# uzh-rpg/dagr

Hardware: AMD Instinct MI355X
Metric: events_per_sec (higher is better)
Workload: dtype f32; 1 GPU; dagr-s + --use_image --img_net resnet50, 640x480 synthetic S-uniform, B=8 windows/step x 100000 events (50 ms each), r=7, K=16, events->graph->GNN(+image fusion)->decoded head outputs->confidence mask + NMS (device); image_branch=in-line, engines=3

## Files before the change

dagr_amd/csrc/gemm_split_bf16.hip:

```cpp
#include <algorithm>
#include <type_traits>

#include "common.hpp"

namespace dagr {
namespace {

constexpr int kKT = 32;
constexpr int kNPad = 128;

typedef __bf16 bf16x8 __attribute__((ext_vector_type(8)));
typedef float f32x4 __attribute__((ext_vector_type(4)));
typedef unsigned u32x2 __attribute__((ext_vector_type(2)));

struct Geo {
    int mode;
    int H, W, C, s, Ho, Wo;
};

struct Args {
    const float *A;
    const unsigned short *Wp;
    const float *bias, *R;
    float *D;
    int64_t M, lda, ldr, ldd;
    int K, N, Npad, act, n_tiles_n, n_blocks;
    Geo g;
};

__device__ __forceinline__ unsigned short bf16_bits(__bf16 v) { return __builtin_bit_cast(unsigned short, v); }

__device__ __forceinline__ void split3(float a, unsigned short &p1, unsigned short &p2, unsigned short &p3) {
    const __bf16 b1 = (__bf16)a;
    const float r1 = a - (float)b1;
    const __bf16 b2 = (__bf16)r1;
    const float r2 = r1 - (float)b2;
    const __bf16 b3 = (__bf16)r2;
    p1 = bf16_bits(b1);
    p2 = bf16_bits(b2);
    p3 = bf16_bits(b3);
}

__device__ __forceinline__ void split3x2(float a0, float a1, unsigned &p1, unsigned &p2, unsigned &p3) {
    typedef float f32x2 __attribute__((ext_vector_type(2)));
    typedef __bf16 bf16x2 __attribute__((ext_vector_type(2)));
    auto widen = [](unsigned u) {
        return f32x2{__builtin_bit_cast(float, u << 16), __builtin_bit_cast(float, u & 0xffff0000u)};
    };
    const f32x2 v = {a0, a1};
    p1 = __builtin_bit_cast(unsigned, __builtin_convertvector(v, bf16x2));
    const f32x2 r1 = v - widen(p1);
    p2 = __builtin_bit_cast(unsigned, __builtin_convertvector(r1, bf16x2));
    const f32x2 r2 = r1 - widen(p2);
    p3 = __builtin_bit_cast(unsigned, __builtin_convertvector(r2, bf16x2));
}

__device__ __forceinline__ int swz(int r, int c) { return r * kKT + ((c ^ (((r >> 3) & 1) * 3)) << 3); }

__global__ __launch_bounds__(256) void k_split_pack(const float *__restrict__ Wt, int K, int N, int Npad,
                                                    unsigned short *__restrict__ out) {
    const int64_t total = (int64_t)K * Npad;
    for (int64_t i = (int64_t)blockIdx.x * blockDim.x + threadIdx.x; i < total; i += (int64_t)gridDim.x * blockDim.x) {
        const int k = (int)(i / Npad), n = (int)(i - (int64_t)k * Npad);
        unsigned short p[3] = {0, 0, 0};
        if (n < N) split3(Wt[(int64_t)k * N + n], p[0], p[1], p[2]);
        const int kt = k / kKT, kk = k - kt * kKT;
#pragma unroll
        for (int q = 0; q < 3; q++) out[((int64_t)kt * 3 + q) * Npad * kKT + swz(n, kk >> 3) + (kk & 7)] = p[q];
    }
}

template <int N>
__device__ __forceinline__ void wait_all_barrier(f32x4 (&ra)[2][N]) {
    if constexpr (N == 1)
        asm volatile("s_waitcnt vmcnt(0) lgkmcnt(0)" : "+v"(ra[0][0]), "+v"(ra[1][0])::"memory");
    else
        asm volatile("s_waitcnt vmcnt(0) lgkmcnt(0)" : "+v"(ra[0][0]), "+v"(ra[0][1]), "+v"(ra[1][0]), "+v"(ra[1][1])::"memory");
    __builtin_amdgcn_s_barrier();
    asm volatile("" ::: "memory");
}

constexpr int waves_per_simd(int BN, int WN) { return WN == 4 ? 4 : BN == 128 ? 2 : 3; }

template <int MI, int BN, int MODE, int WN = 2>
__global__ __launch_bounds__(128 * WN, waves_per_simd(BN, WN)) void k_gemm_split(const Args a) {
    constexpr int BM = 32 * MI;
    constexpr int NT = 128 * WN;
    constexpr int NI = BN / (16 * WN);
    constexpr int AI = BM * 8 / NT;
    constexpr int kStage = 3 * (BM + BN) * kKT;
    constexpr int kPieces = 3 * BN / 16 / (2 * WN);
    static_assert(AI >= 1 && AI * NT == BM * 8 && kPieces * 2 * WN * 16 == 3 * BN && NI >= 1, "tile does not divide among the waves");
    __shared__ __attribute__((aligned(1024))) unsigned short lds[2 * kStage];

    const int orig = blockIdx.x, xcd = orig & 7, q8 = a.n_blocks >> 3, r8 = a.n_blocks & 7;
    const int lid = (xcd < r8 ? xcd * (q8 + 1) : r8 * (q8 + 1) + (xcd - r8) * q8) + (orig >> 3);
    const int nt = lid % a.n_tiles_n, mt = lid / a.n_tiles_n;
    const int64_t m0 = (int64_t)mt * BM;
    const int n0 = nt * BN;

    const int t = threadIdx.x, lane = t & 63, wave = t >> 6;
    const int wm = wave / WN, wn = wave % WN;

    constexpr int kRS = NT / 8;
    const int r0 = t >> 3, c4 = t & 7;
    int64_t rowoff[MODE == 1 ? AI : 1];
    int ryx[MODE == 2 ? AI : 1];
    const int64_t mrow0 = m0 + r0;
    rowoff[0] = (mrow0 < a.M ? mrow0 : 0) * a.lda;
    ryx[0] = 0;
#pragma unroll
    for (int i = 0; i < AI; i++) {
        const int64_t m = mrow0 + kRS * i;
        const int64_t mm = m < a.M ? m : 0;
        if (MODE == 1) {
            const int64_t b = mm / ((int64_t)a.g.Ho * a.g.Wo);
            const int rem = (int)(mm - b * (int64_t)a.g.Ho * a.g.Wo);
            const int yo = rem / a.g.Wo, xo = rem - yo * a.g.Wo;
            rowoff[MODE == 1 ? i : 0] = ((b * a.g.H + (int64_t)yo * a.g.s) * a.g.W + (int64_t)xo * a.g.s) * a.lda;
        } else if (MODE == 2) {
            ryx[MODE == 2 ? i : 0] = (int)((mm / a.g.W) % a.g.H) << 16 | (int)(mm % a.g.W);
        }
    }

    static_assert(AI == 1 || AI == 2, "wait_all_barrier names the register sets");
    f32x4 ra[2][AI];
    unsigned okmask[2] = {0, 0};

    auto gload = [&](auto set, int kt) {
        constexpr int S = decltype(set)::value;
        const int k0 = kt * kKT;
        int c0 = k0, dy = 0, dx = 0;
        int64_t toff = 0;
        if (MODE == 2) {
            const int tap = k0 / a.g.C;
            c0 = k0 - tap * a.g.C;
            dy = tap / 3 - 1;
            dx = tap - (tap / 3) * 3 - 1;
            toff = (int64_t)(dy * a.g.W + dx) * a.lda;
        }
        okmask[S] = 0;
#pragma unroll
        for (int i = 0; i < AI; i++) {
            bool ok = mrow0 + kRS * i < a.M;
            if (MODE == 2) {
                const int yx = ryx[MODE == 2 ? i : 0];
                ok = ok && (unsigned)((yx >> 16) + dy) < (unsigned)a.g.H && (unsigned)((yx & 0xffff) + dx) < (unsigned)a.g.W;
            }
            const int64_t off = MODE == 1 ? rowoff[MODE == 1 ? i : 0] : rowoff[0] + (int64_t)(kRS * i) * a.lda;
            const float *p = ok ? a.A + off + toff + c0 + c4 * 4 : a.A;
            ra[S][i] = *reinterpret_cast<const f32x4 *>(p);
            okmask[S] |= (ok ? 1u : 0u) << i;
        }
    };

    auto lwrite = [&](auto set, int s) {
        constexpr int S = decltype(set)::value;
        unsigned short *const ldsA = lds + s * kStage;
#pragma unroll
        for (int i = 0; i < AI; i++) {
            const bool ok = (okmask[S] >> i) & 1u;
            const f32x4 v = ok ? ra[S][i] : f32x4{0.f, 0.f, 0.f, 0.f};
            unsigned lo[3], hi[3];
            split3x2(v[0], v[1], lo[0], lo[1], lo[2]);
            split3x2(v[2], v[3], hi[0], hi[1], hi[2]);
#pragma unroll
            for (int q = 0; q < 3; q++) {
                const u32x2 u = {lo[q], hi[q]};
                *reinterpret_cast<u32x2 *>(ldsA + q * BM * kKT + swz(r0 + kRS * i, c4 >> 1) + (c4 & 1) * 4) = u;
            }
        }
    };

    const char *const wsrc = reinterpret_cast<const char *>(a.Wp) + ((int64_t)n0 * kKT) * 2 + lane * 16;
    auto wload = [&](int kt, int s) {
#pragma unroll
        for (int j = 0; j < kPieces; j++) {
            const int piece = wave * kPieces + j, p = piece / (BN / 16), sub = piece - p * (BN / 16);
            const char *src = wsrc + (((int64_t)kt * 3 + p) * a.Npad * kKT + sub * 16 * kKT) * 2;
            unsigned short *dst = lds + s * kStage + (3 * BM + p * BN + sub * 16) * kKT;
            __builtin_amdgcn_global_load_lds((const __attribute__((address_space(1))) void *)src,
                                             (__attribute__((address_space(3))) void *)dst, 16, 0, 0);
        }
    };

    f32x4 acc[MI][NI];
#pragma unroll
    for (int mi = 0; mi < MI; mi++)
#pragma unroll
        for (int ni = 0; ni < NI; ni++) acc[mi][ni] = f32x4{0.f, 0.f, 0.f, 0.f};

    const int frag = swz(lane & 15, lane >> 4);
    const int fragA = (wm * 16 * MI) * kKT + frag;
    const int fragW = (3 * BM + wn * (BN / WN)) * kKT + frag;

    const int n_kt = a.K / kKT;
    const std::integral_constant<int, 0> set0;
    const std::integral_constant<int, 1> set1;

    auto multiply = [&](const unsigned short *st) {
        bf16x8 bw[3][NI], av[MI][3];
#pragma unroll
        for (int p = 0; p < 3; p++)
#pragma unroll
            for (int ni = 0; ni < NI; ni++)
                bw[p][ni] = *reinterpret_cast<const bf16x8 *>(st + fragW + (p * BN + ni * 16) * kKT);
#pragma unroll
        for (int mi = 0; mi < MI; mi++)
#pragma unroll
            for (int p = 0; p < 3; p++) av[mi][p] = *reinterpret_cast<const bf16x8 *>(st + fragA + (p * BM + mi * 16) * kKT);
        const f32x4 zero = {0.f, 0.f, 0.f, 0.f};
#pragma unroll
        for (int mi = 0; mi < MI; mi++) {
            f32x4 ts[NI];
#pragma unroll
            for (int ni = 0; ni < NI; ni++) ts[ni] = __builtin_amdgcn_mfma_f32_16x16x32_bf16(bw[2][ni], av[mi][0], zero, 0, 0, 0);
#pragma unroll
            for (int ni = 0; ni < NI; ni++) ts[ni] = __builtin_amdgcn_mfma_f32_16x16x32_bf16(bw[0][ni], av[mi][2], ts[ni], 0, 0, 0);
#pragma unroll
            for (int ni = 0; ni < NI; ni++) ts[ni] = __builtin_amdgcn_mfma_f32_16x16x32_bf16(bw[1][ni], av[mi][1], ts[ni], 0, 0, 0);
#pragma unroll
            for (int ni = 0; ni < NI; ni++) ts[ni] = __builtin_amdgcn_mfma_f32_16x16x32_bf16(bw[1][ni], av[mi][0], ts[ni], 0, 0, 0);
#pragma unroll
            for (int ni = 0; ni < NI; ni++) ts[ni] = __builtin_amdgcn_mfma_f32_16x16x32_bf16(bw[0][ni], av[mi][1], ts[ni], 0, 0, 0);
#pragma unroll
            for (int ni = 0; ni < NI; ni++) ts[ni] = __builtin_amdgcn_mfma_f32_16x16x32_bf16(bw[0][ni], av[mi][0], ts[ni], 0, 0, 0);
#pragma unroll
            for (int ni = 0; ni < NI; ni++) acc[mi][ni] += ts[ni];
        }
    };

    auto slice = [&](auto cur, auto nxt, int kt) {
        constexpr int S = decltype(cur)::value;
        gload(cur, kt + 2 < n_kt ? kt + 2 : n_kt - 1);
        wload(kt + 1, S ^ 1);
        __builtin_amdgcn_sched_barrier(0);
        multiply(lds + S * kStage);
        lwrite(nxt, S ^ 1);
#pragma unroll
        for (int i = 0; i < 6 * MI * NI; i++) {
            __builtin_amdgcn_sched_group_barrier(0x008, 1, 0);
            __builtin_amdgcn_sched_group_barrier(0x002, 3, 0);
        }
        wait_all_barrier(ra);
    };

    gload(set0, 0);
    gload(set1, n_kt > 1 ? 1 : 0);
    wload(0, 0);
    lwrite(set0, 0);
    wait_all_barrier(ra);
    int kt = 0;
    for (; kt + 2 < n_kt; kt += 2) {
        slice(set0, set1, kt);
        slice(set1, set0, kt + 1);
    }
    if (kt + 1 < n_kt) {
        slice(set0, set1, kt);
        kt++;
    }
    multiply(lds + (kt & 1) * kStage);

#pragma unroll
    for (int mi = 0; mi < MI; mi++) {
        const int64_t m = m0 + wm * 16 * MI + mi * 16 + (lane & 15);
        if (m >= a.M) continue;
#pragma unroll
        for (int ni = 0; ni < NI; ni++) {
            const int n = n0 + wn * (BN / WN) + ni * 16 + (lane >> 4) * 4;
            if (n >= a.N) continue;
            f32x4 v = acc[mi][ni];
            if (a.bias) {
                const float4 b = *reinterpret_cast<const float4 *>(a.bias + n);
                v += f32x4{b.x, b.y, b.z, b.w};
            }
            if (a.R) {
                const float4 r = *reinterpret_cast<const float4 *>(a.R + m * a.ldr + n);
                v += f32x4{r.x, r.y, r.z, r.w};
            }
            if (a.act) v = f32x4{fmaxf(v[0], 0.f), fmaxf(v[1], 0.f), fmaxf(v[2], 0.f), fmaxf(v[3], 0.f)};
            *reinterpret_cast<float4 *>(a.D + m * a.ldd + n) = make_float4(v[0], v[1], v[2], v[3]);
        }
    }
}

inline bool aligned16(const void *p) { return ((uintptr_t)p & 15) == 0; }

template <int MI, int BN, int MODE, int WN = 2>
int launch_tile(Args &a, hipStream_t stream) {
    a.n_tiles_n = (int)ceil_div(a.N, BN);
    const int64_t blocks = ceil_div(a.M, 32 * MI) * a.n_tiles_n;
    DAGR_CHECK_ARG(blocks < ((int64_t)1 << 31), "too many tiles");
    a.n_blocks = (int)blocks;
    k_gemm_split<MI, BN, MODE, WN><<<(unsigned)blocks, 128 * WN, 0, stream>>>(a);
    DAGR_CHECK_LAUNCH();
    return DAGR_OK;
}

template <int MODE>
int launch(Args &a, int variant, hipStream_t stream) {
    if (variant == 0) {
        const int64_t cus = device_cu_count();
        if (MODE != 2 && a.K <= 512 && a.N % 128 == 0 && ceil_div(a.M, 64) * (a.N / 128) >= 4 * cus)
            variant = DAGR_SPLIT_64X128_W8;
        else
            variant = ceil_div(a.M, 64) * ceil_div(a.N, 64) >= 2 * cus ? DAGR_SPLIT_64X64 : DAGR_SPLIT_32X64;
    }
    switch (variant) {
        case DAGR_SPLIT_64X128: return launch_tile<2, 128, MODE>(a, stream);
        case DAGR_SPLIT_32X128: return launch_tile<1, 128, MODE>(a, stream);
        case DAGR_SPLIT_64X64: return launch_tile<2, 64, MODE>(a, stream);
        case DAGR_SPLIT_32X64: return launch_tile<1, 64, MODE>(a, stream);
        case DAGR_SPLIT_64X128_W8: return launch_tile<2, 128, MODE, 4>(a, stream);
    }
    set_error("split-bf16 GEMM: unknown variant");
    return DAGR_ERR_INVALID_ARG;
}

inline int unsupported(const char *fn, const char *what) {
    set_error(std::string(fn) + ": " + what);
    return DAGR_ERR_UNSUPPORTED;
}

}
}

using namespace dagr;

extern "C" size_t dagr_gemm_split_bf16_packed_bytes(int32_t K, int32_t N) {
    if (K < kKT || K % kKT != 0 || N < 16 || N % 16 != 0) return 0;
    return (size_t)K * 3 * align_up((size_t)N, kNPad) * sizeof(unsigned short);
}

extern "C" int dagr_gemm_split_bf16_pack(const float *Wt, int32_t K, int32_t N, void *packed, size_t packed_bytes,
                                         void *stream) {
    DAGR_CHECK_ARG(K >= 1 && N >= 1, "bad sizes");
    if (K % kKT != 0) return unsupported(__func__, "K is not a multiple of the K-tile (32)");
    if (N % 16 != 0) return unsupported(__func__, "N is not a multiple of 16");
    DAGR_CHECK_ARG(Wt && packed, "NULL pointer");
    DAGR_CHECK_ARG(aligned16(packed), "packed is not 16-byte aligned");
    DAGR_CHECK_ARG(packed_bytes >= dagr_gemm_split_bf16_packed_bytes(K, N), "packed buffer too small");
    const int Npad = (int)align_up((size_t)N, kNPad);
    const int64_t blocks = std::min<int64_t>(ceil_div((int64_t)K * Npad, 256), 256 * 16);
    k_split_pack<<<(unsigned)blocks, 256, 0, (hipStream_t)stream>>>(Wt, K, N, Npad, (unsigned short *)packed);
    DAGR_CHECK_LAUNCH();
    return DAGR_OK;
}

namespace {
#define SPLIT_CHECK(cond, msg)                                     \
    do {                                                           \
        if (!(cond)) {                                             \
            set_error(std::string(fn) + ": " + (msg));             \
            return DAGR_ERR_INVALID_ARG;                           \
        }                                                          \
    } while (0)

int check_common(const char *fn, const float *A, int64_t M, int32_t K, int64_t lda, const void *packed, int32_t N,
                 const float *bias, const float *R, int64_t ldr, int32_t act, float *D, int64_t ldd, int32_t code,
                 int32_t max_code, bool &done) {
    done = true;
    SPLIT_CHECK(M >= 0 && K >= 1 && N >= 1 && ldd >= N && (!R || ldr >= N) && (act == 0 || act == 1) && code >= 0 &&
                    code <= max_code,
                "bad sizes");
    if (K % kKT != 0) return unsupported(fn, "K (C of a 3x3) is not a multiple of the K-tile (32)");
    if (N % 16 != 0) return unsupported(fn, "N is not a multiple of 16");
    if (M == 0) return DAGR_OK;
    SPLIT_CHECK(A && packed && D, "NULL pointer");
    SPLIT_CHECK((const float *)D != A, "D aliases A");
    SPLIT_CHECK((const float *)D != R, "D aliases R");
    SPLIT_CHECK(lda % 4 == 0 && ldd % 4 == 0 && (!R || ldr % 4 == 0), "row strides must be multiples of 4 floats");
    SPLIT_CHECK(aligned16(A) && aligned16(packed) && aligned16(D) && aligned16(bias) && aligned16(R),
                "pointers must be 16-byte aligned");
    done = false;
    return DAGR_OK;
}

int gemm_entry(const char *fn, const float *A, int64_t M, int32_t K, int64_t lda, const void *packed, int32_t N,
               const float *bias, const float *R, int64_t ldr, int32_t act, float *D, int64_t ldd, int32_t B, int32_t H,
               int32_t W, int32_t stride, int32_t code, int32_t max_code, void *stream) {
    bool done;
    const int rc = check_common(fn, A, M, K, lda, packed, N, bias, R, ldr, act, D, ldd, code, max_code, done);
    if (done) return rc;
    SPLIT_CHECK(lda >= K && stride >= 1, "bad sizes");
    Args a{A, (const unsigned short *)packed, bias, R, D, M, lda, R ? ldr : 0, ldd, K, N, (int)align_up((size_t)N, kNPad), act,
           0, 0, Geo{0, 0, 0, K, 1, 0, 0}};
    if (stride == 1) return launch<0>(a, code, (hipStream_t)stream);
    SPLIT_CHECK(B >= 1 && H >= 1 && W >= 1, "bad image sizes");
    const int Ho = (H - 1) / stride + 1, Wo = (W - 1) / stride + 1;
    SPLIT_CHECK(M == (int64_t)B * Ho * Wo, "M is not B * ceil(H / stride) * ceil(W / stride)");
    a.g = Geo{1, H, W, K, stride, Ho, Wo};
    return launch<1>(a, code, (hipStream_t)stream);
}

int conv3x3_entry(const char *fn, const float *X, int32_t B, int32_t H, int32_t W, int32_t C, int64_t ldx, const void *packed,
                  int32_t N, const float *bias, const float *R, int64_t ldr, int32_t act, float *D, int64_t ldd, int32_t code,
                  int32_t max_code, void *stream) {
    SPLIT_CHECK(B >= 0 && H >= 1 && W >= 1 && C >= 1 && ldx >= C, "bad sizes");
    const int64_t M = (int64_t)B * H * W;
    bool done;
    const int rc = check_common(fn, X, M, C, ldx, packed, N, bias, R, ldr, act, D, ldd, code, max_code, done);
    if (done) return rc;
    SPLIT_CHECK((int64_t)C * 9 < ((int64_t)1 << 31), "C too large");
    Args a{X, (const unsigned short *)packed, bias, R, D, M, ldx, R ? ldr : 0, ldd, 9 * C, N, (int)align_up((size_t)N, kNPad), act,
           0, 0, Geo{2, H, W, C, 1, H, W}};
    return launch<2>(a, code, (hipStream_t)stream);
}
#undef SPLIT_CHECK
}

extern "C" int dagr_gemm_split_bf16(const float *A, int64_t M, int32_t K, int64_t lda, const void *packed, int32_t N,
                                    const float *bias, const float *R, int64_t ldr, int32_t act, float *D, int64_t ldd,
                                    int32_t B, int32_t H, int32_t W, int32_t stride, int32_t tile, void *stream) {
    return gemm_entry(__func__, A, M, K, lda, packed, N, bias, R, ldr, act, D, ldd, B, H, W, stride, tile, 4, stream);
}

extern "C" int dagr_conv3x3_split_bf16(const float *X, int32_t B, int32_t H, int32_t W, int32_t C, int64_t ldx,
                                       const void *packed, int32_t N, const float *bias, const float *R, int64_t ldr,
                                       int32_t act, float *D, int64_t ldd, int32_t tile, void *stream) {
    return conv3x3_entry(__func__, X, B, H, W, C, ldx, packed, N, bias, R, ldr, act, D, ldd, tile, 4, stream);
}

extern "C" int dagr_gemm_split_bf16_variant(const float *A, int64_t M, int32_t K, int64_t lda, const void *packed, int32_t N,
                                            const float *bias, const float *R, int64_t ldr, int32_t act, float *D,
                                            int64_t ldd, int32_t B, int32_t H, int32_t W, int32_t stride, int32_t variant,
                                            void *stream) {
    return gemm_entry(__func__, A, M, K, lda, packed, N, bias, R, ldr, act, D, ldd, B, H, W, stride, variant,
                      DAGR_SPLIT_VARIANT_LAST, stream);
}

extern "C" int dagr_conv3x3_split_bf16_variant(const float *X, int32_t B, int32_t H, int32_t W, int32_t C, int64_t ldx,
                                               const void *packed, int32_t N, const float *bias, const float *R,
                                               int64_t ldr, int32_t act, float *D, int64_t ldd, int32_t variant,
                                               void *stream) {
    return conv3x3_entry(__func__, X, B, H, W, C, ldx, packed, N, bias, R, ldr, act, D, ldd, variant,
                         DAGR_SPLIT_VARIANT_LAST, stream);
}
```

dagr_amd/engine.py:

```python
import contextlib
import ctypes
import gc
import types

import numpy as np
import torch

from . import _lib
from .graph.ev_graph import WindowGraphBuilder

FUSED_PASSES_MAX_NODES = 1600

L0_WIDTHS = (8, 16, 32)


def _l0_block(c):
    cm = max(b for b in (0,) + L0_WIDTHS if b <= c)
    return cm, c - cm


def _f32(v):
    return float(torch.as_tensor(v, dtype=torch.float32))


def _same_domain(a, b):
    return (a["rx"], a["ry"], a["den_x"], a["den_y"]) == (b["rx"], b["ry"], b["den_x"], b["den_y"]) \
        and torch.equal(a["remap"], b["remap"])


def _bn_affine(bn):
    m = bn.module
    scale = (m.weight / torch.sqrt(m.running_var + m.eps)).detach().float()
    shift = (m.bias - m.running_mean * scale).detach().float()
    return scale, shift



@contextlib.contextmanager
def _capture(graph):
    was_enabled = gc.isenabled()
    with torch.cuda.graph(graph):
        gc.disable()
        try:
            yield
        finally:
            if was_enabled:
                gc.enable()

class _ConvPack:

    def __init__(self, cin, cskip, Wm, bias, relu):
        self.K, self.N = Wm.shape
        self.ldw = (self.N + 7) // 8 * 8
        if self.ldw != self.N:
            Wm = torch.cat([Wm, torch.zeros((self.K, self.ldw - self.N), dtype=Wm.dtype, device=Wm.device)], 1)
        self.cin, self.cskip, self.Wm, self.bias, self.relu = cin, cskip, Wm.contiguous(), bias.contiguous(), relu
        K16, N16 = (self.K + 15) // 16 * 16, (self.N + 15) // 16 * 16
        Wp = torch.zeros((K16, N16), dtype=Wm.dtype, device=Wm.device)
        Wp[: self.K, : self.N] = Wm[:, : self.N]
        self.Wq = Wp.view(K16 // 16, 4, 4, N16 // 16, 16).permute(3, 0, 2, 4, 1).contiguous()


def _pack_generic(convs, norms, skip=None, relu=True, device="cuda"):
    cols, biases = [], []
    cin = convs[0].in_channels
    for conv, norm in zip(convs, norms):
        W = conv.weight.detach().float()
        root = conv.lin.weight.detach().float()
        cout = W.shape[2]
        if norm is not None:
            scale, shift = _bn_affine(norm)
        else:
            scale, shift = torch.ones(cout, device=W.device), torch.zeros(cout, device=W.device)
        if conv.bias is not None:
            shift = shift + conv.bias.detach().float() * scale
        block = torch.cat([W.reshape(25 * cin, cout), root.t()], 0) * scale.view(1, -1)
        if skip is not None:
            lin, norm_skip = skip
            s_scale, s_shift = _bn_affine(norm_skip)
            block = torch.cat([block, lin.mlp.weight.detach().float().t() * s_scale.view(1, -1)], 0)
            shift = shift + s_shift
        cols.append(block)
        biases.append(shift)
    cskip = skip[0].mlp.in_features if skip is not None else 0
    return _ConvPack(cin, cskip, torch.cat(cols, 1).to(device), torch.cat(biases).to(device), relu)


def _pack_l0(conv, norm, win, skip=None, device="cuda", cols_in=None, cols_skip=None):
    win_x, tx, win_y, ty = win
    W = conv.weight.detach().float()
    cin, cout = W.shape[1], W.shape[2]
    if cout not in L0_WIDTHS:
        raise NotImplementedError(f"the level-0 kernels exist for {', '.join(map(str, L0_WIDTHS))} output channels "
                                  f"(base_width = 0.25, 0.5, 1.0), not {cout}")
    cols_in = list(range(cin)) if cols_in is None else list(cols_in)
    scale, shift = _bn_affine(norm)
    rows = []
    for b in range(ty):
        for a in range(tx):
            rows.append(W[(win_x + a) + 5 * (win_y + b)][cols_in] * scale.view(1, -1))
    rows.append(conv.lin.weight.detach().float().t()[cols_in] * scale.view(1, -1))
    cskip = 0
    if skip is not None:
        lin, norm_skip = skip
        s_scale, s_shift = _bn_affine(norm_skip)
        ws = lin.mlp.weight.detach().float().t()
        if cols_skip is not None:
            ws = ws[list(cols_skip)]
        rows.append(ws * s_scale.view(1, -1))
        shift = shift + s_shift
        cskip = lin.mlp.in_features
    return cin, cskip, torch.cat(rows, 0).contiguous().to(device), shift.contiguous().to(device)


class _Conv1x1Gemm(torch.nn.Module):

    def __init__(self, conv, relu=False):
        super().__init__()
        cout, cin = conv.weight.shape[:2]
        self.stride = conv.stride[0]
        self.relu = relu
        self.register_buffer("wt", conv.weight.detach().reshape(cout, cin).t().contiguous())
        self.register_buffer("b", conv.bias.detach().clone() if conv.bias is not None else torch.zeros(cout, device=conv.weight.device))
        self.planes = None
        self.path = None

    def forward(self, x, residual=None):
        N = self.wt.shape[1]
        r = None if residual is None else residual.permute(0, 2, 3, 1)
        if self.planes is not None:
            y = _split_conv(x, self.planes, 1, self.stride, N, self.b, r, self.relu or r is not None)
            if y is not None:
                self.path = "split"
                return y
        self.path = "library"
        if self.stride != 1:
            x = x[:, :, ::self.stride, ::self.stride]
        B, C, H, W = x.shape
        a = x.permute(0, 2, 3, 1).reshape(-1, C)
        if _LT["ok"] and a.is_cuda and a.dtype == torch.float32 and a.stride(1) == 1 \
                and (r is None or (r.is_contiguous() and tuple(r.shape) == (B, H, W, N))):
            y = torch.empty((a.shape[0], N), dtype=torch.float32, device=a.device)
            ws = _lt_workspace(a.device)
            act = 1 if (self.relu or r is not None) else 0
            rc = _lib.lib().dagr_gemm_epilogue(_lib.ptr(a), a.shape[0], C, a.stride(0), _lib.ptr(self.wt), N,
                                               _lib.ptr(self.b), _lib.ptr(r), N, act, _lib.ptr(y), N, _lib.ptr(ws),
                                               ws.numel(), _lib.cur_stream(a.device))
            if rc == 0:
                return y.view(B, H, W, -1).permute(0, 3, 1, 2)
            _LT["ok"] = False
        if residual is not None:
            y = torch.addmm(self.b, a, self.wt).view(B, H, W, -1).permute(0, 3, 1, 2)
            return _add_relu_(y, residual)
        y = torch._addmm_activation(self.b, a, self.wt) if self.relu else torch.addmm(self.b, a, self.wt)
        return y.view(B, H, W, -1).permute(0, 3, 1, 2)


_LT = {"ok": True, "ws": {}}


def _lt_workspace(device):
    key = str(device)
    if key not in _LT["ws"]:
        _LT["ws"][key] = torch.empty(int(_lib.lib().dagr_gemm_epilogue_workspace_bytes()), dtype=torch.uint8, device=device)
    return _LT["ws"][key]


def _split_min_rows(K, N, taps):
    if taps == 1:
        if K < 64 or N < 64:
            return None
        if K < 128 or N < 128:
            return 153600 if (K, N) in ((64, 64), (256, 64), (64, 256)) else None
        if K <= 256:
            return 512
        if K <= 512:
            return 2400 if N >= 256 else 38400
        return {(1024, 512): 9600, (1024, 2048): 2400}.get((K, N))
    if taps == 9 and K == N:
        return {64: 153600, 128: 32768, 256: 9600}.get(K)
    return None


def _split_pack(wt):
    L = _lib.lib()
    K, N = wt.shape
    nbytes = int(L.dagr_gemm_split_bf16_packed_bytes(K, N))
    if nbytes == 0 or not wt.is_cuda:
        return None
    out = torch.empty(nbytes, dtype=torch.uint8, device=wt.device)
    _lib.check(L.dagr_gemm_split_bf16_pack(_lib.ptr(wt), K, N, _lib.ptr(out), nbytes, _lib.cur_stream(wt.device)),
               "gemm_split_bf16_pack")
    return out


def _split_conv(x, planes, taps, stride, N, bias, r, relu):
    B, C, H, W = x.shape
    Ho, Wo = (H - 1) // stride + 1, (W - 1) // stride + 1
    M = B * Ho * Wo
    rows = _split_min_rows(C, N, taps)
    xn = x.permute(0, 2, 3, 1)
    if rows is None or M < rows or not (x.is_cuda and x.dtype == torch.float32 and xn.is_contiguous()) \
            or (r is not None and not (r.is_contiguous() and tuple(r.shape) == (B, Ho, Wo, N))):
        return None
    y = torch.empty((B, Ho, Wo, N), dtype=torch.float32, device=x.device)
    L, st = _lib.lib(), _lib.cur_stream(x.device)
    if taps == 1:
        rc = L.dagr_gemm_split_bf16(_lib.ptr(xn), M, C, C, _lib.ptr(planes), N, _lib.ptr(bias), _lib.ptr(r), N, int(relu),
                                    _lib.ptr(y), N, B, H, W, stride, 0, st)
    else:
        rc = L.dagr_conv3x3_split_bf16(_lib.ptr(xn), B, H, W, C, C, _lib.ptr(planes), N, _lib.ptr(bias), _lib.ptr(r), N,
                                       int(relu), _lib.ptr(y), N, 0, st)
    _lib.check(rc, "gemm_split_bf16")
    return y.permute(0, 3, 1, 2)


def _gemmify_1x1(module):
    for name, child in list(module.named_children()):
        if isinstance(child, torch.nn.Conv2d) and child.kernel_size == (1, 1) and child.groups == 1 \
                and child.padding == (0, 0) and child.stride[0] == child.stride[1]:
            setattr(module, name, _Conv1x1Gemm(child))
        else:
            _gemmify_1x1(child)


def _add_relu_(y, z):
    if y.is_cuda and y.dtype == torch.float32 and z.dtype == torch.float32 and y.shape == z.shape \
            and y.stride() == z.stride() and y.data_ptr() % 16 == 0 and z.data_ptr() % 16 == 0 \
            and (y.is_contiguous() or y.is_contiguous(memory_format=torch.channels_last)):
        _lib.check(_lib.lib().dagr_add_relu(_lib.ptr(y), _lib.ptr(z), y.numel(), _lib.cur_stream(y.device)), "add_relu")
        return y
    return torch.relu_(y.add_(z))


def _bias_relu_(y, bias):
    C = y.shape[1]
    if y.is_cuda and y.dtype == torch.float32 and C % 4 == 0 and y.is_contiguous(memory_format=torch.channels_last) \
            and y.data_ptr() % 16 == 0 and bias.data_ptr() % 16 == 0:
        _lib.check(_lib.lib().dagr_bias_relu(_lib.ptr(y), _lib.ptr(bias), y.numel(), C, _lib.cur_stream(y.device)),
                   "bias_relu")
        return y
    return torch.relu_(y.add_(bias.view(1, -1, 1, 1)))


def _baseconv_forward(m, x):
    y = m.conv(x)
    b = m._bias
    C = y.shape[1]
    if y.is_cuda and y.dtype == torch.float32 and C % 4 == 0 and y.is_contiguous(memory_format=torch.channels_last) \
            and y.data_ptr() % 16 == 0 and b.data_ptr() % 16 == 0:
        _lib.check(_lib.lib().dagr_bias_silu(_lib.ptr(y), _lib.ptr(b), y.numel(), C, _lib.cur_stream(y.device)),
                   "bias_silu")
        return y
    return torch.nn.functional.silu(y.add_(b.view(1, -1, 1, 1)), inplace=True)


def _conv_bias_relu(blk, name, x):
    conv = getattr(blk, name)
    b = getattr(blk, "_" + name + "_bias", None)
    planes = getattr(conv, "_split_planes", None)
    if planes is not None:
        out = _split_conv(x, planes, 9, 1, conv.out_channels, b, None, True)
        if out is not None:
            conv._split_path = "split"
            return out
    if isinstance(conv, torch.nn.Conv2d):
        conv._split_path = "library"
    out = conv(x)
    if b is not None:
        return _bias_relu_(out, b)
    if getattr(conv, "relu", False):
        return out
    return blk.relu(out)


def _bottleneck_forward(blk, x):
    identity = x if blk.downsample is None else blk.downsample(x)
    out = _conv_bias_relu(blk, "conv1", x)
    out = _conv_bias_relu(blk, "conv2", out)
    if isinstance(blk.conv3, _Conv1x1Gemm):
        return blk.conv3(out, residual=identity)
    return _add_relu_(blk.conv3(out), identity)


def _resnet_features_forward(net, x, emit=None):
    emit = emit or (lambda name, t: None)
    c1 = net.conv1(x)
    emit("conv1", c1)
    mp = net.maxpool
    ok = (c1.is_cuda and c1.dtype == torch.float32 and c1.is_contiguous(memory_format=torch.channels_last)
          and c1.shape[1] % 4 == 0 and mp.kernel_size == 3 and mp.stride == 2 and mp.padding == 1
          and mp.dilation == 1 and not mp.ceil_mode)
    if ok:
        B, C, H, W = c1.shape
        scale, shift = net._stem_affine
        y = torch.empty((B, C, (H - 1) // 2 + 1, (W - 1) // 2 + 1), dtype=c1.dtype, device=c1.device,
                        memory_format=torch.channels_last)
        _lib.check(_lib.lib().dagr_bn_relu_maxpool(_lib.ptr(c1), B, H, W, C, _lib.ptr(scale), _lib.ptr(shift), _lib.ptr(y),
                                                   _lib.cur_stream(c1.device)), "bn_relu_maxpool")
    else:
        y = net.maxpool(net.relu(net.bn1(c1)))
    l1 = net.layer1(y)
    emit("layer1", l1)
    l2 = net.layer2(l1)
    emit("layer2", l2)
    l3 = net.layer3(l2)
    emit("layer3", l3)
    l4 = net.layer4(l3)
    emit("layer4", l4)
    return dict(conv1=c1, layer1=l1, layer2=l2, layer3=l3, layer4=l4)


def _basicblock_forward(blk, x):
    identity = x if blk.downsample is None else blk.downsample(x)
    out = _conv_bias_relu(blk, "conv1", x)
    return _add_relu_(blk.conv2(out), identity)


def flicker_map_bytes(B, sensor_w, sensor_h):
    pixels = B * sensor_w * sensor_h
    return 2 * (-(-8 * pixels // 256) * 256) + 4 * pixels


def flicker_maps_from_state(state, B, sensor_w, sensor_h):
    pixels, shape = B * sensor_w * sensor_h, (B, sensor_h, sensor_w)
    stride = -(-8 * pixels // 256) * 256
    t_edge = state[:8 * pixels].view(torch.int64).cpu().numpy().reshape(shape)
    t_pass = state[stride:stride + 8 * pixels].view(torch.int64).cpu().numpy().reshape(shape)
    word = state[2 * stride:2 * stride + 4 * pixels].view(torch.int32).cpu().numpy().reshape(shape)
    polarity = np.array([0, 1, -1, 0], np.int8)
    return dict(t_edge=t_edge, last_p=polarity[(word >> 9) & 3], count=(word & 0xff).astype(np.int32),
                blocking=((word >> 8) & 1).astype(bool), t_pass=t_pass, p_pass=polarity[(word >> 11) & 3])


class StreamState:

    def __init__(self, batch_size, window_us, device, max_lane_events=None):
        self.B, self.window_us, self.device = int(batch_size), int(window_us), torch.device(device)
        self.max_lane_events = None if max_lane_events is None else int(max_lane_events)
        self.lane_dropped = torch.zeros((self.B,), dtype=torch.int64, device=self.device)
        self.cap = 0
        self.state = None
        self.status = torch.zeros((1,), dtype=torch.int32, device=self.device)
        self.lane_count = torch.zeros((self.B,), dtype=torch.int32, device=self.device)
        self.image = None
        self.frame_new = True
        self.frame_steps = self.held_steps = 0
        self._host = torch.zeros((self.B,), dtype=torch.int32).pin_memory()
        self._known = np.zeros((self.B,), np.int64)
        self._since = 0
        self._fresh = True
        self.front = None
        self.front_state, self.front_cap, self.front_out = None, 0, None
        self.noise = None
        self.noise_state, self.noise_cap, self.noise_out, self.lane_filtered = None, 0, None, None
        self.flick = None
# ... 814 lines not shown
    def forward_append(self, pos, feat, batch, static_out=False):
        if not self.l0_tiles:
            raise NotImplementedError("asynchronous updates run on the tiled level-0 conv (16 neighbours, 3x3/3x5 tap window)")
        L, P = self.L, _lib.ptr
        if not self._async_on:
            self.async_begin()
        n = int(pos.shape[0])
        a = self._app
        first = self._n_rows
        stream = _lib.cur_stream(self.device)
        if n:
            self._grow_rows(first + n)
            a = self._app
            pos = pos.float().contiguous()
            feat = feat.float().reshape(-1).contiguous()
            batch = batch.contiguous()
        if not self.use_image:
            self._async_call(a, first, n, pos if n else None, feat if n else None, batch if n else None, stream)
            self._n_rows = first + n
        else:
            if n:
                b64 = 1 if batch.dtype == torch.int64 else 0
                g = self.graph
                _lib.check(L.dagr_async_graph_append(ctypes.byref(g.desc), P(g.workspace), self._N, first, P(a["head"]),
                                                     P(a["next"]), P(a["xytb"]), a["next"].shape[0], P(pos), 0, P(batch), b64,
                                                     n, P(self.nbr_src), P(self.nbr_code), P(self.deg), P(a["status"]), P(feat),
                                                     P(self.pos_n), P(self.batch_n), P(a["batch_ev"]), P(self.x0buf),
                                                     self.x0_ld, self.x0_feat_col, self.x0_pos_col, stream),
                           "async_graph_append")
                rows = slice(first, first + n)
                self._sample(None, n, self.pos_n[rows], self.batch_n[rows], 0, self._img_feats[0], self.x0buf[rows],
                             self.x0_img_col)
                c = self.cout0
                self._conv_l0_rows(self.l0_conv1, first, n, P(self.x0buf), self.x0_ld, None, 0, P(self.h1), c)
                self._conv_l0_rows(self.l0_conv2, first, n, P(self.h1), c, P(self.x0buf), self.x0_ld, P(self.hp0),
                                   self.hp0.shape[1])
                self._sample(None, n, self.pos_n[rows], self.batch_n[rows], 0, self._img_feats[1], self.hp0[rows], c)
                self._n_rows = first + n
            self._pool1_stream(rebuild=False, first=first, n=n)
        if self.tail_graph and not self.use_image:
            return self._replay_tail(static_out)
        return self._tail_and_head()

    def _conv_generic(self, lvl, pack, x, ldx, xskip, ldskip, out, ldo, dom, stream, code=None, scratch=None):
        L = self.L
        P = _lib.ptr
        code = lvl.code if code is None else code
        scratch = self.A if scratch is None else scratch
        passes = L.dagr_spline_conv_fused_passes(pack.cin, pack.cskip)
        if passes == 1 or (passes > 1 and lvl.T <= FUSED_PASSES_MAX_NODES):
            _lib.check(L.dagr_spline_conv_fused(P(lvl.counts), lvl.T, P(lvl.rowptr), P(lvl.col), P(code), x, ldx,
                                                pack.cin, xskip, ldskip, pack.cskip, dom["rx"], dom["ry"], dom["den_x"],
                                                dom["den_y"], P(pack.Wq), P(pack.bias), out, ldo, pack.N,
                                                1 if pack.relu else 0, stream), "spline_conv_fused")
            return
        lda = (pack.K + 3) // 4 * 4
        _lib.check(L.dagr_spline_tap_aggregate(P(lvl.counts), lvl.T, P(lvl.rowptr), P(lvl.col), P(code),
                                               x, ldx, pack.cin, xskip, ldskip, pack.cskip, dom["rx"], dom["ry"],
                                               dom["den_x"], dom["den_y"], P(scratch), lda, stream), "tap_aggregate")
        _lib.check(L.dagr_gemm_bias_act(P(lvl.counts), lvl.T, P(scratch), lda, P(pack.Wm), pack.ldw, P(pack.bias),
                                        out, ldo, pack.K, pack.N, 1 if pack.relu else 0, stream), "gemm")

    def stage_graph(self, pos, batch, feat=None):
        N = int(pos.shape[0])
        self._alloc_events(N)
        self._N = N
        self._pos, self._batch = pos, batch
        self._nbr = (self.nbr_src[:N], self.nbr_code[:N], self.deg[:N])
        inputs = None
        if feat is not None and pos.dtype == torch.float32:
            self._feat_flat = feat.float().reshape(-1).contiguous()
            inputs = _lib.L0Inputs(feat=self._feat_flat.data_ptr(), pos_nodes=self.pos_n.data_ptr(),
                                   batch_nodes=self.batch_n.data_ptr(), x0=self.x0buf.data_ptr(), ldx0=self.x0_ld,
                                   col_feat=self.x0_feat_col, col_pos=self.x0_pos_col)
        self.graph.build(pos, batch, out=self._nbr, n_dev=self.n_dev if self._dev_mode else None, inputs=inputs)
        self._inputs_gathered = inputs is not None
        self._n_rows = N
        self._async_on = False

    def _nptr(self):
        return self.graph.node_count_ptr() if self._dev_mode else None

    def _sample(self, n_ptr, n_max, pos, batch, b64, fmap, out, coff):
        if self._feat_ready is not None:
            ready = self._feat_ready.get(id(fmap))
            if ready is None:
                raise RuntimeError("pipelined window: a sampled feature map has no ready-event (the image branch did not "
                                   "announce it) -- reading it would race with the image stream")
            torch.cuda.current_stream(self.device).wait_event(ready)
        Bf, C, h, w = fmap.shape
        nhwc = fmap.permute(0, 2, 3, 1)
        if not nhwc.is_contiguous():
            nhwc = nhwc.contiguous()
        self._keep.append(nhwc)
        _lib.check(self.L.dagr_sample_features(n_ptr, n_max, _lib.ptr(pos), _lib.ptr(batch), b64, _lib.ptr(nhwc), Bf, h,
                                               w, C, self.W, self.H, _lib.ptr(out), out.shape[1], coff,
                                               _lib.cur_stream(self.device)), "sample_features")

    def _fold_image_branch(self):
        import copy
        from torch.nn.utils.fusion import fuse_conv_bn_eval
        bb, head = self.model.backbone, self.model.head
        net = copy.deepcopy(bb.net).eval()
        cnn = copy.deepcopy(head.cnn_head).eval()

        def fold_block(blk):
            for ci, bi in (("conv1", "bn1"), ("conv2", "bn2"), ("conv3", "bn3")):
                if hasattr(blk, ci):
                    setattr(blk, ci, fuse_conv_bn_eval(getattr(blk, ci), getattr(blk, bi)))
                    setattr(blk, bi, torch.nn.Identity())
            if blk.downsample is not None:
                blk.downsample = torch.nn.Sequential(fuse_conv_bn_eval(blk.downsample[0], blk.downsample[1]))
        for name in ("layer1", "layer2", "layer3", "layer4"):
            for blk in getattr(net.module, name):
                fold_block(blk)
        for m in cnn.modules():
            if hasattr(m, "conv") and hasattr(m, "bn") and isinstance(m.bn, torch.nn.BatchNorm2d):
                m.conv = fuse_conv_bn_eval(m.conv, m.bn)
                m.bn = torch.nn.Identity()
                if isinstance(getattr(m, "act", None), torch.nn.SiLU) and m.conv.bias is not None:
                    m._bias = m.conv.bias.detach().clone().contiguous()
                    m.conv.bias = None
                    m.forward = types.MethodType(_baseconv_forward, m)
        net = net.to(memory_format=torch.channels_last)
        cnn = cnn.to(memory_format=torch.channels_last)
        for blkname in ("layer1", "layer2", "layer3", "layer4"):
            _gemmify_1x1(getattr(net.module, blkname))
            for blk in getattr(net.module, blkname):
                relu_convs = ("conv1", "conv2") if hasattr(blk, "conv3") else ("conv1",)
                for cname in relu_convs:
                    conv = getattr(blk, cname)
                    if isinstance(conv, _Conv1x1Gemm):
                        conv.relu = True
                    elif isinstance(conv, torch.nn.Conv2d) and conv.bias is not None:
                        setattr(blk, "_" + cname + "_bias", conv.bias.detach().clone().contiguous())
                        conv.bias = None
                        if conv.kernel_size == (3, 3) and conv.stride == (1, 1) and conv.padding == (1, 1) \
                                and conv.dilation == (1, 1) and conv.groups == 1 \
                                and _split_min_rows(conv.in_channels, conv.out_channels, 9) is not None:
                            conv._split_planes = _split_pack(conv.weight.detach().permute(2, 3, 1, 0).reshape(
                                9 * conv.in_channels, conv.out_channels).contiguous())
                for m in blk.modules():
                    if isinstance(m, _Conv1x1Gemm) and _split_min_rows(m.wt.shape[0], m.wt.shape[1], 1) is not None:
                        m.planes = _split_pack(m.wt)
                blk.forward = types.MethodType(_bottleneck_forward if hasattr(blk, "conv3") else _basicblock_forward,
                                               blk)
        bn = net.module.bn1
        scale = (bn.weight.detach().float() / torch.sqrt(bn.running_var.detach().float() + bn.eps)).contiguous()
        shift = (bn.bias.detach().float() - bn.running_mean.detach().float() * scale).contiguous()
        net.module._stem_affine = (scale, shift)
        net.module.forward_features = types.MethodType(_resnet_features_forward, net.module)
        _gemmify_1x1(net.feature_dconv)
        _gemmify_1x1(net.output_dconv)
        self._net_f, self._cnn_f = net, cnn

    def image_branch_paths(self):
        if self._net_f is None:
            return {}
        out = {}
        for name, m in self._net_f.named_modules():
            path = m.path if isinstance(m, _Conv1x1Gemm) else getattr(m, "_split_path", None)
            if path is not None:
                out[name] = path
        return out

    def _image_branch(self, image, on_feature=None):
        if self._net_f is None:
            self._fold_image_branch()
        bb, head = types.SimpleNamespace(net=self._net_f), types.SimpleNamespace(cnn_head=self._cnn_f)
        x = image.contiguous(memory_format=torch.channels_last)
        net = self._net_f
        if on_feature is not None:
            feats = [None] * len(net.feature_layers)

            def emit(name, t):
                if name in net.feature_layers:
                    j = net.feature_layers.index(name)
                    feats[j] = net.feature_dconv[j](t) if len(net.feature_dconv) > 0 else t
                    on_feature(j, feats[j])
            d = _resnet_features_forward(net.module, x, emit)
            outs = [d[l] for l in net.output_layers]
            if len(net.output_dconv) > 0:
                outs = [dconv(o) for o, dconv in zip(outs, net.output_dconv)]
        else:
            feats, outs = bb.net(x)
        outs = outs[-self.num_scales:]
        resized = [torch.nn.functional.interpolate(f, o) for f, o in zip(outs, self.out_sizes)]
        return feats, head.cnn_head(resized)

    def stage_image(self, image):
        self._keep = []
        self._held_for = None
        self._img_feats, self._cnn_out = self._image_branch(image)

    def image_async(self, image, stream=None):
        cur = torch.cuda.current_stream(self.device)
        if stream is not None:
            self._img_stream = stream
        if self._img_stream is None:
            self._img_stream = torch.cuda.Stream(self.device)
        s = self._img_stream
        s.wait_stream(cur)
        with torch.cuda.stream(s):
            feats, cnn_out = self._image_branch(image)
            ev = torch.cuda.Event()
            ev.record(s)
        return feats, cnn_out, ev

    def image_handle_from(self, feats, cnn_out):
        ev = torch.cuda.Event()
        ev.record(torch.cuda.current_stream(self.device))
        return list(feats), cnn_out, ev

    def held_maps(self, st):
        if not self.use_image or self._held_for is not st or st.frame_new:
            return None
        return self._img_feats, self._cnn_out

    def _consume_image_handle(self, handle):
        feats, cnn_out, ev = handle
        cur = torch.cuda.current_stream(self.device)
        cur.wait_event(ev)
        for t in list(feats) + [o for v in cnn_out.values() for o in v]:
            t.record_stream(cur)
        self._keep = []
        self._held_for = None
        self._img_feats, self._cnn_out = feats, cnn_out

    def stage_l0_input(self, feat):
        N = self._N
        x0 = self.x0buf[:N]
        g = self.graph
        if not self._inputs_gathered:
            f = feat.float().reshape(-1).contiguous()
            _lib.check(self.L.dagr_graph_gather_inputs(ctypes.byref(g.desc), _lib.ptr(g.workspace), _lib.ptr(self._pos),
                                                       _lib.ptr(f), N, _lib.ptr(self.pos_n), _lib.ptr(self.batch_n),
                                                       _lib.ptr(x0), self.x0_ld, self.x0_feat_col, self.x0_pos_col,
                                                       _lib.cur_stream(self.device)), "graph_gather_inputs")
        if self.use_image:
            self._sample(self._nptr(), N, self.pos_n, self.batch_n, 0, self._img_feats[0], x0, self.x0_img_col)
        self._x0 = x0

    def _conv_l0(self, pack, x, ldx, xskip, ldskip, out, ldo):
        L, P = self.L, _lib.ptr
        nbr_src, nbr_code, deg = self._nbr
        cin, cskip, w, s = pack
        d0 = self.dom[0]
        wx, tx, wy, ty = self.win0
        stream = _lib.cur_stream(self.device)
        if self.l0_tiles:
            cm, ce = self._l0_blocks[cin]
            _lib.check(L.dagr_spline_conv_l0_tiles_w(self.cout0, cm, ce, cskip, wx, tx, wy, ty, d0["rx"], d0["ry"],
                                                     d0["den_x"], d0["den_y"], self._N, self.graph.K, P(nbr_src), P(nbr_code),
                                                     P(deg), x, ldx, xskip, ldskip, P(w), P(s), 1, out, ldo, self._nptr(),
                                                     stream), "conv_l0_tiles")
        else:
            _lib.check(L.dagr_spline_conv_l0(cin, cskip, self.ntaps0, self._N, self.graph.K, self.ncodes0, P(nbr_src),
                                             P(nbr_code), P(deg), x, ldx, xskip, ldskip, P(self.tab0), P(w), P(s), 1,
                                             out, ldo, stream), "conv_l0")

    def stage_l0_conv1(self):
        P = _lib.ptr
        assert self.l0_conv1[0] == len(self.x0_cols)
        self._conv_l0(self.l0_conv1, P(self._x0), self.x0_ld, None, 0, P(self.h1), self.cout0)

    def stage_l0_conv2(self, sample=True):
        P = _lib.ptr
        self._conv_l0(self.l0_conv2, P(self.h1), self.cout0, P(self._x0), self.x0_ld, P(self.hp0), self.hp0.shape[1])
        if self.use_image and sample:
            self._sample(self._nptr(), self._N, self.pos_n, self.batch_n, 0, self._img_feats[1], self.hp0[:self._N],
                         self.cout0)

    def stage_l0_sample1(self):
        self._sample(None, self._N, self.pos_n, self.batch_n, 0, self._img_feats[1], self.hp0[:self._N], self.cout0)

    def stage_pool1(self):
        L, P = self.L, _lib.ptr
        g = self.graph
        nbr_src, nbr_code, deg = self._nbr
        l1 = self.levels[0]
        d = self.pool_desc[0]
        b64 = 1 if self._batch.dtype == torch.int64 else 0
        _lib.check(L.dagr_pool_l0(ctypes.byref(d), P(self.pool_ws[0]), ctypes.byref(g.desc), P(g.workspace),
                                  P(self.xlo), P(self.ylo), P(self.hp0), self.hp0.shape[1], P(self.pos_n),
                                  P(self.batch_n), P(self._batch), b64, self._N, P(nbr_src),
                                  P(nbr_code) if self.fast_coarse_edges else None, P(deg), P(self.cluster0), P(l1.x),
                                  l1.x.shape[1], 0, P(l1.pos), P(l1.batch), P(l1.counts), P(l1.rowptr), P(l1.col),
                                  P(l1.code), ctypes.c_void_p(l1.counts.data_ptr() + 4), l1.e_cap,
                                  _lib.cur_stream(self.device)), "pool_l0")

    def pool1_accumulate_again(self):
        L, P = self.L, _lib.ptr
        g = self.graph
        nbr_src, nbr_code, deg = self._nbr
        _lib.check(L.dagr_pool_l0_accumulate(ctypes.byref(self.pool_desc[0]), P(self.pool_ws[0]), ctypes.byref(g.desc),
                                             P(g.workspace), P(self.xlo), P(self.ylo), P(self.hp0), self.hp0.shape[1],
                                             P(self.pos_n), self._N, P(nbr_src),
                                             P(nbr_code) if self.fast_coarse_edges else None, P(deg),
                                             _lib.cur_stream(self.device)), "pool_l0_accumulate")

    def _stage_level(self, k, trace=None):
        L, P = self.L, _lib.ptr
        stream = _lib.cur_stream(self.device)
        lvl = self.levels[k]
        c1, c2 = self.packs[k]
        dom = self.dom[k + 1]
# ... 636 lines not shown
```

Measured before the change: 163.3 million events/s.

## Use buffer loads with OOB masking in split-bf16 GEMM and extend to dconv layers

```diff
diff --git a/dagr_amd/csrc/gemm_split_bf16.hip b/dagr_amd/csrc/gemm_split_bf16.hip
--- a/dagr_amd/csrc/gemm_split_bf16.hip
+++ b/dagr_amd/csrc/gemm_split_bf16.hip
@@ -25,8 +25,12 @@
     float *D;
     int64_t M, lda, ldr, ldd;
     int K, N, Npad, act, n_tiles_n, n_blocks;
+    unsigned a_bytes, w_bytes;
     Geo g;
 };
+
+constexpr unsigned kMasked = 0x80000000u;
+constexpr int kRsrcFlags = 0x00020000;
 
 __device__ __forceinline__ unsigned short bf16_bits(__bf16 v) { return __builtin_bit_cast(unsigned short, v); }
 
@@ -78,6 +82,16 @@
         asm volatile("s_waitcnt vmcnt(0) lgkmcnt(0)" : "+v"(ra[0][0]), "+v"(ra[0][1]), "+v"(ra[1][0]), "+v"(ra[1][1])::"memory");
     __builtin_amdgcn_s_barrier();
     asm volatile("" ::: "memory");
+}
+
+template <int I, int N, int V>
+__device__ __forceinline__ void interleave() {
+    if constexpr (I < N) {
+        __builtin_amdgcn_sched_group_barrier(0x008, 1, 0);
+        constexpr int n = (I + 1) * V / N - I * V / N;
+        if constexpr (n > 0) __builtin_amdgcn_sched_group_barrier(0x002, n, 0);
+        interleave<I + 1, N, V>();
+    }
 }
 
 constexpr int waves_per_simd(int BN, int WN) { return WN == 4 ? 4 : BN == 128 ? 2 : 3; }
@@ -99,58 +113,68 @@
     const int64_t m0 = (int64_t)mt * BM;
     const int n0 = nt * BN;
 
-    const int t = threadIdx.x, lane = t & 63, wave = t >> 6;
+    const int t = threadIdx.x, lane = t & 63, wave = __builtin_amdgcn_readfirstlane(t >> 6);
     const int wm = wave / WN, wn = wave % WN;
 
     constexpr int kRS = NT / 8;
     const int r0 = t >> 3, c4 = t & 7;
-    int64_t rowoff[MODE == 1 ? AI : 1];
-    int ryx[MODE == 2 ? AI : 1];
+    unsigned voff[AI];
+    unsigned tapout[MODE == 2 ? AI : 1];
+    tapout[0] = 0;
     const int64_t mrow0 = m0 + r0;
-    rowoff[0] = (mrow0 < a.M ? mrow0 : 0) * a.lda;
-    ryx[0] = 0;
 #pragma unroll
     for (int i = 0; i < AI; i++) {
         const int64_t m = mrow0 + kRS * i;
-        const int64_t mm = m < a.M ? m : 0;
+        const bool ok = m < a.M;
+        const int64_t mm = ok ? m : 0;
+        int64_t pix = mm;
         if (MODE == 1) {
             const int64_t b = mm / ((int64_t)a.g.Ho * a.g.Wo);
             const int rem = (int)(mm - b * (int64_t)a.g.Ho * a.g.Wo);
             const int yo = rem / a.g.Wo, xo = rem - yo * a.g.Wo;
-            rowoff[MODE == 1 ? i : 0] = ((b * a.g.H + (int64_t)yo * a.g.s) * a.g.W + (int64_t)xo * a.g.s) * a.lda;
+            pix = (b * a.g.H + (int64_t)yo * a.g.s) * a.g.W + (int64_t)xo * a.g.s;
         } else if (MODE == 2) {
-            ryx[MODE == 2 ? i : 0] = (int)((mm / a.g.W) % a.g.H) << 16 | (int)(mm % a.g.W);
-        }
-    }
+            const int y = (int)((mm / a.g.W) % a.g.H), x = (int)(mm % a.g.W);
+            unsigned out = 0;
+#pragma unroll
+            for (int tap = 0; tap < 9; tap++) {
+                const int dy = tap / 3 - 1, dx = tap % 3 - 1;
+                const bool in = ok && (unsigned)(y + dy) < (unsigned)a.g.H && (unsigned)(x + dx) < (unsigned)a.g.W;
+                out |= (in ? 0u : 1u) << tap;
+            }
+            tapout[MODE == 2 ? i : 0] = out;
+        }
+        voff[i] = ok ? (unsigned)(pix * a.lda * 4 + c4 * 16) : MODE == 2 ? 0u : kMasked;
+    }
+    const __amdgpu_buffer_rsrc_t arsrc = __builtin_amdgcn_make_buffer_rsrc(const_cast<float *>(a.A), 0, (int)a.a_bytes, kRsrcFlags);
 
     static_assert(AI == 1 || AI == 2, "wait_all_barrier names the register sets");
     f32x4 ra[2][AI];
-    unsigned okmask[2] = {0, 0};
+
+    const int n_kt = a.K / kKT;
+    int nx_kt = 0, nx_c0 = 0, nx_tx = 0;
+    unsigned nx_tapoff = 0, nx_shift = 31;
+    const unsigned pix_bytes = (unsigned)a.lda * 4u;
 
     auto gload = [&](auto set, int kt) {
         constexpr int S = decltype(set)::value;
-        const int k0 = kt * kKT;
-        int c0 = k0, dy = 0, dx = 0;
-        int64_t toff = 0;
+        unsigned soff = (unsigned)kt * (kKT * 4);
+        if (MODE == 2) soff = nx_tapoff + (unsigned)nx_c0 * 4u;
+#pragma unroll
+        for (int i = 0; i < AI; i++) {
+            unsigned v = voff[i];
+            if (MODE == 2) v |= (tapout[MODE == 2 ? i : 0] << nx_shift) & kMasked;
+            ra[S][i] = __builtin_bit_cast(f32x4, __builtin_amdgcn_raw_buffer_load_b128(arsrc, (int)v, (int)soff, 0));
+        }
         if (MODE == 2) {
-            const int tap = k0 / a.g.C;
-            c0 = k0 - tap * a.g.C;
-            dy = tap / 3 - 1;
-            dx = tap - (tap / 3) * 3 - 1;
-            toff = (int64_t)(dy * a.g.W + dx) * a.lda;
-        }
-        okmask[S] = 0;
-#pragma unroll
-        for (int i = 0; i < AI; i++) {
-            bool ok = mrow0 + kRS * i < a.M;
-            if (MODE == 2) {
-                const int yx = ryx[MODE == 2 ? i : 0];
-                ok = ok && (unsigned)((yx >> 16) + dy) < (unsigned)a.g.H && (unsigned)((yx & 0xffff) + dx) < (unsigned)a.g.W;
-            }
-            const int64_t off = MODE == 1 ? rowoff[MODE == 1 ? i : 0] : rowoff[0] + (int64_t)(kRS * i) * a.lda;
-            const float *p = ok ? a.A + off + toff + c0 + c4 * 4 : a.A;
-            ra[S][i] = *reinterpret_cast<const f32x4 *>(p);
-            okmask[S] |= (ok ? 1u : 0u) << i;
+            const bool more = nx_kt + 1 < n_kt;
+            const bool tapstep = more && nx_c0 + kKT == a.g.C;
+            const bool rowstep = tapstep && nx_tx == 2;
+            nx_kt += more ? 1 : 0;
+            nx_c0 = tapstep ? 0 : more ? nx_c0 + kKT : nx_c0;
+            nx_shift -= tapstep ? 1u : 0u;
+            nx_tapoff += rowstep ? (unsigned)(a.g.W - 2) * pix_bytes : tapstep ? pix_bytes : 0u;
+            nx_tx = rowstep ? 0 : tapstep ? nx_tx + 1 : nx_tx;
         }
     };
 
@@ -159,8 +183,7 @@
         unsigned short *const ldsA = lds + s * kStage;
 #pragma unroll
         for (int i = 0; i < AI; i++) {
-            const bool ok = (okmask[S] >> i) & 1u;
-            const f32x4 v = ok ? ra[S][i] : f32x4{0.f, 0.f, 0.f, 0.f};
+            const f32x4 v = ra[S][i];
             unsigned lo[3], hi[3];
             split3x2(v[0], v[1], lo[0], lo[1], lo[2]);
             split3x2(v[2], v[3], hi[0], hi[1], hi[2]);
@@ -172,15 +195,16 @@
         }
     };
 
-    const char *const wsrc = reinterpret_cast<const char *>(a.Wp) + ((int64_t)n0 * kKT) * 2 + lane * 16;
+    const __amdgpu_buffer_rsrc_t wrsrc =
+        __builtin_amdgcn_make_buffer_rsrc(const_cast<unsigned short *>(a.Wp), 0, (int)a.w_bytes, kRsrcFlags);
+    const int wlane = lane * 16;
     auto wload = [&](int kt, int s) {
 #pragma unroll
         for (int j = 0; j < kPieces; j++) {
             const int piece = wave * kPieces + j, p = piece / (BN / 16), sub = piece - p * (BN / 16);
-            const char *src = wsrc + (((int64_t)kt * 3 + p) * a.Npad * kKT + sub * 16 * kKT) * 2;
+            const unsigned soff = (unsigned)(((kt * 3 + p) * a.Npad + n0 + sub * 16) * (kKT * 2));
             unsigned short *dst = lds + s * kStage + (3 * BM + p * BN + sub * 16) * kKT;
-            __builtin_amdgcn_global_load_lds((const __attribute__((address_space(1))) void *)src,
-                                             (__attribute__((address_space(3))) void *)dst, 16, 0, 0);
+            __builtin_amdgcn_raw_ptr_buffer_load_lds(wrsrc, (__attribute__((address_space(3))) void *)dst, 16, wlane, (int)soff, 0, 0);
         }
     };
 
@@ -194,7 +218,6 @@
     const int fragA = (wm * 16 * MI) * kKT + frag;
     const int fragW = (3 * BM + wn * (BN / WN)) * kKT + frag;
 
-    const int n_kt = a.K / kKT;
     const std::integral_constant<int, 0> set0;
     const std::integral_constant<int, 1> set1;
 
@@ -237,11 +260,7 @@
         __builtin_amdgcn_sched_barrier(0);
         multiply(lds + S * kStage);
         lwrite(nxt, S ^ 1);
-#pragma unroll
-        for (int i = 0; i < 6 * MI * NI; i++) {
-            __builtin_amdgcn_sched_group_barrier(0x008, 1, 0);
-            __builtin_amdgcn_sched_group_barrier(0x002, 3, 0);
-        }
+        interleave<0, 6 * MI * NI, 20 * AI + 2 * MI * NI + (MODE == 2 ? 2 * AI + 1 : 0)>();
         wait_all_barrier(ra);
     };
 
@@ -321,6 +340,14 @@
     set_error(std::string(fn) + ": " + what);
     return DAGR_ERR_UNSUPPORTED;
 }
+
+inline int64_t view_bytes(int64_t rows, int64_t ld, int64_t K, int64_t front) {
+    const int64_t lim = (int64_t)1 << 31;
+    if (rows - 1 + front >= lim || ld >= lim) return -1;
+    const int64_t bytes = ((rows - 1 + front) * ld + K) * 4;
+    return bytes < lim ? bytes : -1;
+}
+constexpr const char *kViewTooLarge = "the A view spans 2^31 bytes or more (the kernel addresses it with 32-bit offsets)";
 
 }
 }
@@ -383,14 +410,22 @@
     const int rc = check_common(fn, A, M, K, lda, packed, N, bias, R, ldr, act, D, ldd, code, max_code, done);
     if (done) return rc;
     SPLIT_CHECK(lda >= K && stride >= 1, "bad sizes");
+    const size_t wbytes = dagr_gemm_split_bf16_packed_bytes(K, N);
+    if (wbytes >= ((size_t)1 << 31)) return unsupported(fn, "the packed weights span 2^31 bytes or more");
     Args a{A, (const unsigned short *)packed, bias, R, D, M, lda, R ? ldr : 0, ldd, K, N, (int)align_up((size_t)N, kNPad), act,
-           0, 0, Geo{0, 0, 0, K, 1, 0, 0}};
-    if (stride == 1) return launch<0>(a, code, (hipStream_t)stream);
-    SPLIT_CHECK(B >= 1 && H >= 1 && W >= 1, "bad image sizes");
-    const int Ho = (H - 1) / stride + 1, Wo = (W - 1) / stride + 1;
-    SPLIT_CHECK(M == (int64_t)B * Ho * Wo, "M is not B * ceil(H / stride) * ceil(W / stride)");
-    a.g = Geo{1, H, W, K, stride, Ho, Wo};
-    return launch<1>(a, code, (hipStream_t)stream);
+           0, 0, 0, (unsigned)wbytes, Geo{0, 0, 0, K, 1, 0, 0}};
+    int64_t rows = M;
+    if (stride != 1) {
+        SPLIT_CHECK(B >= 1 && H >= 1 && W >= 1, "bad image sizes");
+        const int Ho = (H - 1) / stride + 1, Wo = (W - 1) / stride + 1;
+        SPLIT_CHECK(M == (int64_t)B * Ho * Wo, "M is not B * ceil(H / stride) * ceil(W / stride)");
+        a.g = Geo{1, H, W, K, stride, Ho, Wo};
+        rows = (int64_t)B * H * W;
+    }
+    const int64_t abytes = view_bytes(rows, lda, K, 0);
+    if (abytes < 0) return unsupported(fn, kViewTooLarge);
+    a.a_bytes = (unsigned)abytes;
+    return stride == 1 ? launch<0>(a, code, (hipStream_t)stream) : launch<1>(a, code, (hipStream_t)stream);
 }
 
 int conv3x3_entry(const char *fn, const float *X, int32_t B, int32_t H, int32_t W, int32_t C, int64_t ldx, const void *packed,
@@ -402,8 +437,12 @@
     const int rc = check_common(fn, X, M, C, ldx, packed, N, bias, R, ldr, act, D, ldd, code, max_code, done);
     if (done) return rc;
     SPLIT_CHECK((int64_t)C * 9 < ((int64_t)1 << 31), "C too large");
-    Args a{X, (const unsigned short *)packed, bias, R, D, M, ldx, R ? ldr : 0, ldd, 9 * C, N, (int)align_up((size_t)N, kNPad), act,
-           0, 0, Geo{2, H, W, C, 1, H, W}};
+    const size_t wbytes = dagr_gemm_split_bf16_packed_bytes(9 * C, N);
+    if (wbytes >= ((size_t)1 << 31)) return unsupported(fn, "the packed weights span 2^31 bytes or more");
+    const int64_t abytes = view_bytes(M, ldx, C, (int64_t)W + 1);
+    if (abytes < 0) return unsupported(fn, kViewTooLarge);
+    Args a{X - ((int64_t)W + 1) * ldx, (const unsigned short *)packed, bias, R, D, M, ldx, R ? ldr : 0, ldd, 9 * C, N,
+           (int)align_up((size_t)N, kNPad), act, 0, 0, (unsigned)abytes, (unsigned)wbytes, Geo{2, H, W, C, 1, H, W}};
     return launch<2>(a, code, (hipStream_t)stream);
 }
 #undef SPLIT_CHECK
diff --git a/dagr_amd/engine.py b/dagr_amd/engine.py
--- a/dagr_amd/engine.py
+++ b/dagr_amd/engine.py
@@ -176,7 +176,7 @@
             return 512
         if K <= 512:
             return 2400 if N >= 256 else 38400
-        return {(1024, 512): 9600, (1024, 2048): 2400}.get((K, N))
+        return {(1024, 256): 9600, (1024, 512): 9600, (1024, 2048): 2400}.get((K, N))
     if taps == 9 and K == N:
         return {64: 153600, 128: 32768, 256: 9600}.get(K)
     return None
@@ -202,6 +202,8 @@
     xn = x.permute(0, 2, 3, 1)
     if rows is None or M < rows or not (x.is_cuda and x.dtype == torch.float32 and xn.is_contiguous()) \
             or (r is not None and not (r.is_contiguous() and tuple(r.shape) == (B, Ho, Wo, N))):
+        return None
+    if ((B * H * W - 1 + (W + 1 if taps == 9 else 0)) * C + C) * 4 >= 1 << 31:
         return None
     y = torch.empty((B, Ho, Wo, N), dtype=torch.float32, device=x.device)
     L, st = _lib.lib(), _lib.cur_stream(x.device)
@@ -1322,6 +1324,10 @@
         net.module.forward_features = types.MethodType(_resnet_features_forward, net.module)
         _gemmify_1x1(net.feature_dconv)
         _gemmify_1x1(net.output_dconv)
+        for dconvs in (net.feature_dconv, net.output_dconv):
+            for m in dconvs.modules():
+                if isinstance(m, _Conv1x1Gemm) and _split_min_rows(m.wt.shape[0], m.wt.shape[1], 1) is not None:
+                    m.planes = _split_pack(m.wt)
         self._net_f, self._cnn_f = net, cnn
 
     def image_branch_paths(self):
```

Measured after the change: 171.0 million events/s, median of 6. +4.7%, better.
